# rockcarry/ffcnn

Measured on AMD Instinct MI355X. Metric: frames/sec yolo-fastest-1.1 @320x320 batch-64 per GPU (u8 BGR frames -> net_input's conversion in the first kernel -> full forward: conv stack + YOLO decode + NMS, boxes on rank 0), higher is better.
Workload: dtype f32

## Files before the change

ffcnn_amd/csrc/ffgpu_conv_kernels.inc:

```
#include "ffgpu_dw_stream.inc"
#include "ffgpu_pw_mfma.inc"
#include "ffgpu_pw_gemm32.inc"
#include "ffgpu_pw_bf16.inc"
#include "ffgpu_conv_igemm.inc"
#include "ffgpu_dwpw.inc"
#include "ffgpu_conv_dense.inc"
#include "ffgpu_irb.inc"
#include "ffgpu_irb_thin.inc"
#include "ffgpu_front.inc"
#include "ffgpu_irb_wave.inc"
#include "ffgpu_irb_wave2.inc"
#include "ffgpu_pw_x3.inc"
#include "ffgpu_pw_x3t.inc"
#include "ffgpu_conv_x3.inc"
#include "ffgpu_dw_lds.inc"
#include "ffgpu_dw_pair.inc"
#include "ffgpu_conv_thin.inc"

struct BareScratch {
    float *p = nullptr; size_t n = 0; int dev = -1;
    float *get(size_t need)
    {
        int d = 0;
        (void)hipGetDevice(&d);
// ... 1079 lines not shown
            const long tiles = (long)((d.OW + 4 * TWq - 1) / (4 * TWq)) * ((d.OH + TH - 1) / TH);
            const double cost = (double)tiles * (NSI * (c.KS1 * 128.0 + 500.0) + 4 * (220.0 + c.OT * 128.0)) * (1.0 + 12.0 / EW);
            if (cost < best) { best = cost; c.TWq = TWq; c.TH = TH; c.EW = EW; c.EH = EH; c.NSI = NSI; }
        }
    }
    if (best > 1e29) return false;
    const int ft = env_int("FFGPU_IRBW_TWQ", 0), fh = env_int("FFGPU_IRBW_TH", 0);
    if (ft > 0 && fh > 0 && ft * fh <= 16) {
        const int EW = S == 1 ? 4 * ft + 4 : 8 * ft + 4, EH = S * (fh - 1) + 3;
        if (EW * EH <= c.NSI * 64) { c.TWq = ft; c.TH = fh; c.EW = EW; c.EH = EH; }
    }
    const long ntiles = (long)d.N * ((d.OW + 4 * c.TWq - 1) / (4 * c.TWq)) * ((d.OH + c.TH - 1) / c.TH);
    const int regs = c.NSI * c.KS1 * 4 + c.OT * 16 + 2 * (c.KS1 + 4 * c.OT) + 76;
    c.big = regs > 124;
    if (env_int("FFGPU_IRBW_BIG", -1) >= 0) c.big = env_int("FFGPU_IRBW_BIG", -1) != 0;
    if (S == 2 && c.KS1 == 1 && env_int("FFGPU_IRBW_BIG_S2K1", -1) >= 0) c.big = env_int("FFGPU_IRBW_BIG_S2K1", -1) != 0;
    const bool conc = (d.flags & FFGPU_CONCURRENT) != 0;
    const int gmax = std::min(8, c.ngroups);
    int G = 1;
    for (int g = 1; g <= gmax; g++) {
        const size_t slot = (size_t)c.OT * 1024, ereg = (size_t)g * 16 * c.NSI * 64;
        if (g > 1 && ereg / slot < (size_t)(g + 1) / 2) continue;
        G = g;
        if (ntiles * g >= env_int("FFGPU_IRBW_GWAVES", conc ? 500 : 1200)) break;
    }
    if (!conc && G > 1 && G < gmax && c.ngroups % G != 0 && (c.ngroups + G) / (G + 1) <= (c.ngroups + G - 1) / G) G++;
    if (d.stride == 1 && c.ngroups == 9 && ntiles >= 400 && ntiles < 512 && gmax >= 4 && !conc && !env_int("FFGPU_IRBW_NOEXC", 0)) G = 4;
    if (ntiles >= 256 && ntiles < 1100 && env_int("FFGPU_IRBW_G_MID", 0) > 0) G = std::min(gmax, env_int("FFGPU_IRBW_G_MID", 0));
    const bool xl_ok = S == 1 && c.KS1 == 12 && c.OT == 3 && c.NSI == 2 && c.big && ((env_int("FFGPU_IRBW_X3", 30) >> 3) & 1) != 0;
    if (xl_ok && conc && ntiles < 256) G = std::min(gmax, env_int("FFGPU_IRBW_G_XL", 7));
    if (ntiles < 256 && env_int("FFGPU_IRBW_G_SMALL", 0) > 0) G = std::min(gmax, env_int("FFGPU_IRBW_G_SMALL", 0));
    const int fg = env_int("FFGPU_IRBW_G", 0);
    if (fg >= 1 && fg <= gmax) G = fg;
    c.G = G;
    c.NSO = 1;
    c.x3 = S == 1 && c.KS1 == 6 && c.OT == 2 && c.NSI == 2 && c.big && ((env_int("FFGPU_IRBW_X3", 30) >> 2) & 1) != 0;
    if (S == 2 && c.KS1 == 4 && c.OT == 2 && c.NSI == 4 && c.big && ((env_int("FFGPU_IRBW_X3", 30) >> 4) & 1) != 0) c.x3 = true;
    c.xl = xl_ok && G > 1;
    if (c.xl) c.x3 = true;
    if (G == 1 && S == 1 && c.OT == 1 && (c.KS1 == 2 || c.KS1 == 4) && env_int("FFGPU_IRBW_NSO", 2) == 2) {
        double best2 = 1e30; int tw2 = 0, th2 = 0;
        for (int TWq = 1; TWq <= 8; TWq++) {
            if (TWq > 1 && (TWq - 1) * 4 >= d.OW) break;
            for (int TH = 1; TWq * TH <= 32 && TH <= d.OH + 1; TH++) {
                if (TWq * TH <= 16 || TWq * ((TH + 1) / 2) > 16) continue;
                const int EW = 4 * TWq + 4, EH = TH + 2;
                if (EW * EH > 192) continue;
                const long tiles = (long)((d.OW + 4 * TWq - 1) / (4 * TWq)) * ((d.OH + TH - 1) / TH);
                const double cost = (double)tiles * (3 * (c.KS1 * 128.0 + 500.0) + 2 * 4 * (220.0 + 128.0)) * (1.0 + 12.0 / EW);
                if (cost < best2) { best2 = cost; tw2 = TWq; th2 = TH; }
            }
        }
        const int f2t = env_int("FFGPU_IRBW2_TWQ", 0), f2h = env_int("FFGPU_IRBW2_TH", 0);
        if (f2t > 0 && f2h > 0 && f2t * ((f2h + 1) / 2) <= 16 && (4 * f2t + 4) * (f2h + 2) <= 192) { tw2 = f2t; th2 = f2h; best2 = 0; }
        const long nt2 = tw2 ? (long)d.N * ((d.OW + 4 * tw2 - 1) / (4 * tw2)) * ((d.OH + th2 - 1) / th2) : 0;
        if (tw2 && best2 < 0.93 * best && nt2 >= env_int("FFGPU_IRBW2_MIN_TILES", 768)) {
            c.NSO = 2; c.TWq = tw2; c.TH = th2; c.EW = 4 * tw2 + 4; c.EH = th2 + 2; c.NSI = 3; c.big = true; c.WPB = 4; c.xl = false;
            c.x3 = irbw_x3_has(c.KS1) && ((env_int("FFGPU_IRBW_X3", 30) >> (c.KS1 == 2 ? 0 : 1)) & 1) != 0;
        }
    }
    {
        const size_t cs = ((size_t)c.ngroups * 224 + c.OT * 32) * sizeof(float), slice = (size_t)16 * c.NSI * 64 * sizeof(float);
        const int cap = c.big ? 12 : 16;
        const int w4 = std::min(cap, (int)(IRB_LDS_MAX / (cs + 4 * slice)) * 4), w8 = std::min(cap, (int)(IRB_LDS_MAX / (cs + 8 * slice)) * 8);
        c.WPB = G > 1 ? G : (w4 >= w8 ? 4 : 8);
        const int fw = env_int("FFGPU_IRBW_WPB", 0);
        if (G == 1 && fw >= 1 && fw <= 8) c.WPB = fw;
    }
    return true;
}

static int irbw_half(const IrbDesc &d, const IrbwCfg &c)
{
    const int r = d.ec & 15;
    const bool on = d.half ? d.half == 2 : env_int("FFGPU_IRBW_HALF", 1) != 0;
    return c.NSO == 1 && r >= 1 && r <= 8 && on ? 1 : 0;
}

static void irbw_layout(const IrbwCfg &c, int &o_w2, int &o_cs, int &cs_floats, int &total)
{
    o_w2 = c.x3 ? c.ngroups * irbw_x3_nm(c.KS1) * 256 : c.ngroups * c.KS1 * 64;
    o_cs = o_w2 + c.ngroups * 4 * c.OT * 64;
    cs_floats = c.ngroups * 16 * 14 + c.OT * 32;
    total = o_cs + cs_floats;
}

template <typename L>
static int irbw_traced(const IrbwP &p, long nblocks, hipStream_t s, L launch)
{
    {
        static unsigned long long *d_t = nullptr;
        if (!d_t && hipMalloc(&d_t, 4096 * 16 * sizeof(unsigned long long)) != hipSuccess) return -1;
        IrbwP q = p; q.dbg_t = d_t;
        (void)hipMemsetAsync(d_t, 0, 4096 * 16 * sizeof(unsigned long long), s);
        launch(q);
        (void)hipStreamSynchronize(s);
        const long nb = std::min(nblocks, 4096L);
        std::vector<unsigned long long> h((size_t)nb * 16);
        (void)hipMemcpy(h.data(), d_t, h.size() * sizeof(unsigned long long), hipMemcpyDeviceToHost);
        unsigned long long t0 = ~0ull, t1 = 0; double d[5] = { 0 }, ex[6] = { 0 }; double late = 0;
        for (long b = 0; b < nb; b++) { t0 = std::min(t0, h[b * 16]); t1 = std::max(t1, h[b * 16 + 5]); }
        for (long b = 0; b < nb; b++) {
            late = std::max(late, (double)(h[b * 16] - t0) * 0.01);
            d[0] += (double)(h[b * 16 + 1] - h[b * 16]) / nb * 0.01; d[1] += (double)(h[b * 16 + 2] - h[b * 16 + 1]) / nb * 0.01;
            d[2] += (double)(h[b * 16 + 3] - h[b * 16 + 2]) / nb * 0.01;
            const unsigned long long t4 = h[b * 16 + 4] ? h[b * 16 + 4] : h[b * 16 + 3];
            d[3] += (double)(t4 - h[b * 16 + 3]) / nb * 0.01; d[4] += (double)(h[b * 16 + 5] - t4) / nb * 0.01;
            for (int k = 0; k < 6; k++) ex[k] += (double)h[b * 16 + 8 + k] / nb * 0.01;
        }
        fprintf(stderr, "  trace irbw %dx%d %d->%d->%d: span %.2f us (first %ld blocks), last start +%.2f | issue loads %.2f barrier %.2f groups %.2f [expand mfma %.2f store %.2f dw0 %.2f prj0 %.2f dw1 %.2f prj1 %.2f] reduce %.2f rows %.2f (us, wave 0, mean per workgroup)\n",
                p.W, p.H, p.ic, p.ec, p.oc, (double)(t1 - t0) * 0.01, nb, late, d[0], d[1], d[2], ex[0], ex[1], ex[2], ex[3], ex[4], ex[5], d[3], d[4]);
        return 0;
    }
}

template <int KS1, int OT, int S, int NSI, bool BIG>
static int irbw_launch_t(const IrbwP &p, size_t lds, long nblocks, int threads, hipStream_t s)
{
    if (lds_allow((const void *)k_irbw<KS1, OT, S, NSI, BIG>, lds, "irbw")) return -1;
    if (env_int("FFGPU_IRB_TRACE", 0))
        return irbw_traced(p, nblocks, s, [&](const IrbwP &q) { hipLaunchKernelGGL((k_irbw<KS1, OT, S, NSI, BIG>), dim3((unsigned)nblocks), dim3(threads), lds, s, q); });
    hipLaunchKernelGGL((k_irbw<KS1, OT, S, NSI, BIG>), dim3((unsigned)nblocks), dim3(threads), lds, s, p);
    LAUNCH_OK("irbw");
    return 0;
}

static int launch_irbw(const IrbDesc &d, const IrbwCfg &c, hipStream_t s)
{
    auto slope = [](int act) { return act == 2 ? 0.1f : (act == 1 ? 0.f : 1.f); };
    IrbwP p;
    p.in = d.in; p.out = d.out; p.residual = d.residual; p.pk = d.pk;
    p.N = d.N; p.H = d.H; p.W = d.W; p.OH = d.OH; p.OW = d.OW; p.ic = d.ic; p.ec = d.ec; p.oc = d.oc;
    p.act1 = slope(d.act1); p.actd = slope(d.actd); p.act2 = slope(d.act2); p.res_act = slope(d.res_act);
    p.TWq = c.TWq; p.TH = c.TH; p.EW = c.EW; p.EH = c.EH;
    p.tiles_x = (d.OW + 4 * c.TWq - 1) / (4 * c.TWq); p.tiles_y = (d.OH + c.TH - 1) / c.TH;
    p.ntiles = (long)d.N * p.tiles_x * p.tiles_y;
    p.ngroups = c.ngroups; p.G = c.G; p.WPB = c.WPB;
    p.half_last = irbw_half(d, c);
    { const int x = env_int("FFGPU_IRBW_XCD", 3); p.xcd = c.G > 1 ? (x >> 1) & 1 : x & 1; }
    int total;
    irbw_layout(c, p.o_w2, p.o_cs, p.cs_floats, total);
    size_t region = (size_t)(c.G > 1 ? c.G : c.WPB) * 16 * c.NSI * 64;
    if (c.G > 1 && !env_int("FFGPU_IRBW_FOLD", 0)) {
        const size_t want = (size_t)c.G * c.OT * 1024;
        if (want > region && (p.cs_floats + want) * sizeof(float) <= 150 * 1024 && p.ntiles <= 512) region = want;
    }
    p.red_cap = (int)(region / ((size_t)c.OT * 1024));
    p.in_elems = (unsigned)((size_t)d.ic * d.N * d.H * d.W);
    p.vec = d.OW % 4 == 0 ? 4 : (d.OW % 2 == 0 ? 2 : 1);
    p.m_ew = (unsigned)(((1ULL << 32) + c.EW - 1) / c.EW);
    {
        auto magic = [](long dv) { return dv <= 1 ? 0u : (unsigned)(((1ULL << 32) + (unsigned long long)dv - 1) / (unsigned long long)dv); };
        if (p.ntiles * std::max(p.tiles_x, p.tiles_y) >= (1L << 32) || p.ntiles >= (1L << 31)) { ffgpu_set_error("irbw: too many tiles for 32-bit index arithmetic"); return -1; }
        p.m_tx = magic(p.tiles_x); p.m_ty = magic(p.tiles_y); p.m_twq = magic(p.TWq);
    }
    p.dbg_t = nullptr;
    const int waves = c.G > 1 ? c.G : c.WPB;
    p.xl_off = (int)((size_t)p.cs_floats + region);
    const size_t lds = ((size_t)p.cs_floats + region + (c.xl ? (size_t)c.NSI * 4 * 64 * IRBW_XL_DW : 0)) * sizeof(float);
    const long nblocks = c.G > 1 ? p.ntiles : (p.ntiles + c.WPB - 1) / c.WPB;
    if (env_int("FFGPU_VERBOSE_IRB", 0))
        fprintf(stderr, "irbw %dx%d %d->%d->%d s%d: tile %dx%d halo %dx%d (%d strips, %d out), %d groups, G %d, %ld tiles, %ld blocks x %d waves, lds %zu B%s\n",
                d.W, d.H, d.ic, d.ec, d.oc, d.stride, 4 * c.TWq, c.TH, c.EW, c.EH, c.NSI, c.NSO, c.ngroups, c.G, p.ntiles, nblocks, waves, lds, c.big ? ", 256 VGPR" : "");
    if (c.NSO == 2) {
        if (c.KS1 == 2 && c.x3)  { hipLaunchKernelGGL((k_irbw2<2, 3, true>), dim3((unsigned)nblocks), dim3(waves * 64), lds, s, p); LAUNCH_OK("irbw2"); return 0; }
        if (c.KS1 == 4 && c.x3)  { hipLaunchKernelGGL((k_irbw2<4, 3, true>), dim3((unsigned)nblocks), dim3(waves * 64), lds, s, p); LAUNCH_OK("irbw2"); return 0; }
        if (c.KS1 == 2) { hipLaunchKernelGGL((k_irbw2<2, 3, false>), dim3((unsigned)nblocks), dim3(waves * 64), lds, s, p); LAUNCH_OK("irbw2"); return 0; }
        if (c.KS1 == 4) { hipLaunchKernelGGL((k_irbw2<4, 3, false>), dim3((unsigned)nblocks), dim3(waves * 64), lds, s, p); LAUNCH_OK("irbw2"); return 0; }
    }
    if (c.xl && c.NSO == 1) {
        if (lds_allow((const void *)k_irbw<12, 3, 1, 2, true, true, true>, lds, "irbw")) return -1;
        if (env_int("FFGPU_IRB_TRACE", 0))
            return irbw_traced(p, nblocks, s, [&](const IrbwP &q) { hipLaunchKernelGGL((k_irbw<12, 3, 1, 2, true, true, true>), dim3((unsigned)nblocks), dim3(waves * 64), lds, s, q); });
        hipLaunchKernelGGL((k_irbw<12, 3, 1, 2, true, true, true>), dim3((unsigned)nblocks), dim3(waves * 64), lds, s, p);
        LAUNCH_OK("irbw");
        return 0;
    }
    if (c.x3 && c.NSO == 1 && c.KS1 == 4 && c.OT == 2 && d.stride == 2 && c.NSI == 4) {
        if (lds_allow((const void *)k_irbw<4, 2, 2, 4, true, true>, lds, "irbw")) return -1;
        if (env_int("FFGPU_IRB_TRACE", 0))
            return irbw_traced(p, nblocks, s, [&](const IrbwP &q) { hipLaunchKernelGGL((k_irbw<4, 2, 2, 4, true, true>), dim3((unsigned)nblocks), dim3(waves * 64), lds, s, q); });
        hipLaunchKernelGGL((k_irbw<4, 2, 2, 4, true, true>), dim3((unsigned)nblocks), dim3(waves * 64), lds, s, p);
        LAUNCH_OK("irbw");
        return 0;
    }
    if (c.x3 && c.NSO == 1 && c.KS1 == 6 && c.OT == 2 && d.stride == 1 && c.NSI == 2) {
        if (lds_allow((const void *)k_irbw<6, 2, 1, 2, true, true>, lds, "irbw")) return -1;
        if (env_int("FFGPU_IRB_TRACE", 0))
            return irbw_traced(p, nblocks, s, [&](const IrbwP &q) { hipLaunchKernelGGL((k_irbw<6, 2, 1, 2, true, true>), dim3((unsigned)nblocks), dim3(waves * 64), lds, s, q); });
        hipLaunchKernelGGL((k_irbw<6, 2, 1, 2, true, true>), dim3((unsigned)nblocks), dim3(waves * 64), lds, s, p);
        LAUNCH_OK("irbw");
        return 0;
    }
#define IRBW_CASE(ks1, ot, st, nsi) if (c.KS1 == ks1 && c.OT == ot && d.stride == st && c.NSI == nsi) \
        return c.big ? irbw_launch_t<ks1, ot, st, nsi, true>(p, lds, nblocks, waves * 64, s) : irbw_launch_t<ks1, ot, st, nsi, false>(p, lds, nblocks, waves * 64, s);
    IRBW_CASE(1, 1, 1, 2); IRBW_CASE(2, 1, 1, 2); IRBW_CASE(4, 1, 1, 2); IRBW_CASE(2, 2, 1, 2); IRBW_CASE(4, 2, 1, 2); IRBW_CASE(6, 2, 1, 2); IRBW_CASE(12, 3, 1, 2);
// ... 55 lines not shown
    LAUNCH_OK("front");
    return 0;
}

bool ffgpu_irb_supported(const IrbDesc &d)
{
    if (irb_thin_ok(d)) return true;
    { IrbwCfg c; if (irbw_pick(d, c)) return true; }
    if (d.stride != 1 && d.stride != 2) return false;
    if (d.oc > 48 || d.ic > 64 || d.ec < 1) return false;
    if (d.act1 == 3 || d.actd == 3 || d.act2 == 3 || d.res_act == 3) return false;
    if (((long)d.H * d.W) % 4 || ((long)d.OH * d.OW) % 4) return false;
    IrbP p;
    return irb_pick_tile(d, p);
}

static void irb_consts(const IrbDesc &d, int &k4, int &ECH, int &MT, int &OT, int &nchunks, int &CH)
{
    k4 = (d.ic + 3) & ~3; OT = (d.oc + 15) / 16;
    ECH = irb_ech(d); MT = ECH / 16;
    nchunks = (d.ec + ECH - 1) / ECH;
    CH = irb_chunk_floats(k4, ECH, OT);
}

size_t ffgpu_irb_pack_floats(const IrbDesc &d)
{
    if (irb_thin_ok(d)) return 64;
    { IrbwCfg c; if (irbw_pick(d, c)) { int a, b, cs, total; irbw_layout(c, a, b, cs, total); return (size_t)total; } }
    int k4, ECH, MT, OT, nchunks, CH;
    irb_consts(d, k4, ECH, MT, OT, nchunks, CH);
    return ((size_t)nchunks * CH + OT * 32 + 63) & ~(size_t)63;
}

void ffgpu_irb_plan(IrbDesc &d) { d.half = env_int("FFGPU_IRBW_HALF", 1) != 0 ? 2 : 1; }

int ffgpu_irb_pack(const IrbDesc &d, float *pk, hipStream_t s)
{
    if (irb_thin_ok(d)) return 0;
    { IrbwCfg c;
      if (irbw_pick(d, c)) {
          int a, b, cs, total; irbw_layout(c, a, b, cs, total);
          IrbwPackP q; q.w1 = d.w1; q.wd = d.wd; q.w2 = d.w2; q.pk = pk; q.ic = d.ic; q.ec = d.ec; q.oc = d.oc;
          q.k4 = (d.ic + 3) & ~3; q.OT = c.OT; q.ngroups = c.ngroups; q.x3 = c.x3 ? 1 : 0; q.half = irbw_half(d, c);
          hipLaunchKernelGGL(k_irbw_pack, dim3((total + 255) / 256), dim3(256), 0, s, q);
          LAUNCH_OK("irbw_pack");
          return 0;
      } }
    IrbPackP q;
    q.w1 = d.w1; q.wd = d.wd; q.w2 = d.w2; q.pk = pk;
    q.ic = d.ic; q.ec = d.ec; q.oc = d.oc;
    irb_consts(d, q.k4, q.ECH, q.MT, q.OT, q.nchunks, q.CH);
    const int total = q.nchunks * q.CH + q.OT * 32;
    hipLaunchKernelGGL(k_irb_pack, dim3((total + 255) / 256), dim3(256), 0, s, q);
    LAUNCH_OK("irb_pack");
    return 0;
}

template <int MT, int OT, int S, int SPW, int NW>
static int irb_launch_t(const IrbP &p, size_t lds, long nblocks, hipStream_t s)
{
    if (lds_allow((const void *)k_irb<MT, OT, SPW, S, NW>, lds, "irb")) return -1;
    if (env_int("FFGPU_IRB_TRACE", 0)) {
        static unsigned long long *d_t = nullptr;
        if (!d_t && hipMalloc(&d_t, 4096 * 16 * sizeof(unsigned long long)) != hipSuccess) return -1;
        IrbP q = p; q.dbg_t = d_t;
        (void)hipMemsetAsync(d_t, 0, 4096 * 16 * sizeof(unsigned long long), s);
        hipLaunchKernelGGL((k_irb<MT, OT, SPW, S, NW>), dim3((unsigned)nblocks), dim3(NW * 64), lds, s, q);
        (void)hipStreamSynchronize(s);
        std::vector<unsigned long long> h((size_t)nblocks * 16);
        (void)hipMemcpy(h.data(), d_t, h.size() * sizeof(unsigned long long), hipMemcpyDeviceToHost);
        unsigned long long t0 = ~0ull, t1 = 0; double d[7] = { 0 }, ph[4] = { 0 };
        for (long b = 0; b < nblocks; b++) {
            t0 = std::min(t0, h[b * 16]); t1 = std::max(t1, h[b * 16 + 7]);
            for (int k = 0; k < 7; k++) d[k] += (double)(h[b * 16 + k + 1] - h[b * 16 + k]) / nblocks * 0.01;
            for (int k = 0; k < 4; k++) ph[k] += (double)h[b * 16 + 8 + k] / nblocks * 0.01;
        }
// ... 61 lines not shown
```

ffcnn_amd/csrc/ffgpu_dev.hpp:

```cpp
#pragma once
#include <hip/hip_runtime.h>
#include <stddef.h>
#include <stdint.h>
#include <vector>
#include "ffgpu_internal.h"

#define FFGPU_CHECK(expr)                                                                   \
    do {                                                                                    \
        hipError_t e_ = (expr);                                                             \
        if (e_ != hipSuccess) {                                                             \
            ffgpu_set_error("%s failed: %s (%s:%d)", #expr, hipGetErrorString(e_), __FILE__, __LINE__); \
            return -1;                                                                      \
        }                                                                                   \
    } while (0)

struct ConvDesc {
    const float *in;
    const float *const *in_ind;
    const float *filt;
    float       *out;
    const float *residual;
    const float *wpack;
    int   N;
    int   iw, ih, ic;
    int   ow, oh, oc;
    int   fs, stride, pad, groups;
    int   act;
    int   res_act;
    int   flags;
    long  in_cs, in_ns, out_cs, out_ns, res_cs, res_ns;
    int   nsplit;
    int   kernel;
    int   x3_mt;
};
#define FFGPU_F_BATCH_INPUT (1 << 30)

static inline int conv_k4(const ConvDesc &d) { return (d.fs * d.fs * (d.ic / d.groups) + 3) & ~3; }

struct IrbDesc {
    const float *in; float *out; const float *residual;
    const float *w1, *wd, *w2;
    int N, H, W, OH, OW, ic, ec, oc, stride;
    int act1, actd, act2, res_act;
    const float *pk;
    int flags;
    int half;
};
bool   ffgpu_irb_supported(const IrbDesc &d);
bool   ffgpu_irb_is_thin(const IrbDesc &d);
size_t ffgpu_irb_pack_floats(const IrbDesc &d);
void   ffgpu_irb_plan(IrbDesc &d);
int    ffgpu_irb_pack(const IrbDesc &d, float *pk, hipStream_t s);
int    ffgpu_launch_irb(const IrbDesc &d, hipStream_t s);
bool   ffgpu_front_ok(const ConvDesc &c, const IrbDesc &d);
enum InputForm { IN_F32, IN_U8, IN_BGR_FRAMES, IN_NV12_FRAMES, IN_FORMS };
int    ffgpu_launch_front(const ConvDesc &c, const IrbDesc &d, InputForm form, hipStream_t s);
bool   ffgpu_front_nv12_fused();
int    ffgpu_front_nc(const IrbDesc &d);

bool   ffgpu_dwpw_ok(const ConvDesc &dw, const ConvDesc &pw);
size_t ffgpu_dwpw_pack_floats(const ConvDesc &dw, const ConvDesc &pw);
int    ffgpu_dwpw_pack(const ConvDesc &dw, const ConvDesc &pw, float *pk, hipStream_t s);
int    ffgpu_launch_dwpw(const ConvDesc &dw, const ConvDesc &pw, const float *wpack, hipStream_t s);

size_t ffgpu_pw_pack_floats(const ConvDesc &d);
void   ffgpu_conv_plan(ConvDesc &d);
int    ffgpu_pw_pack(const ConvDesc &d, float *pk, hipStream_t s);

struct FrameDesc {
    const unsigned char *bgr;
    int w, h, pitch;
    int sw, sh, s1, s2;
    int fmt;
    const unsigned char *uv;
    int pitch_uv;
    int pad_;
};
static_assert(sizeof(FrameDesc) == 56, "FrameDesc: 64 of them travel by value as k_set_frames' argument");
#define FFGPU_YUV_MATRICES { { 16, 298, 409, 100, 208, 516 }, { 0, 256, 359, 88, 183, 454 }, { 16, 298, 459, 55, 136, 541 }, { 0, 256, 403, 48, 120, 475 } }
// ... 50 lines not shown
```

ffcnn_amd/csrc/ffgpu_irb_wave.inc:

```
typedef float v4f_w __attribute__((ext_vector_type(4)));
typedef float v2f_w __attribute__((ext_vector_type(2)));

struct IrbwP {
    const float *in; float *out; const float *residual;
    const float *pk;
    int N, H, W, OH, OW, ic, ec, oc;
    float act1, actd, act2, res_act;
    int TWq, TH, EW, EH;
    int tiles_x, tiles_y;
    long ntiles;
    int ngroups, G, WPB;
    int o_w2, o_cs;
    int cs_floats;
    int xl_off;
    int red_cap;
    unsigned in_elems;
    int vec;
    int half_last;
    unsigned m_ew;
    unsigned m_tx, m_ty, m_twq;
    int xcd;
    unsigned long long *dbg_t;
};

__device__ __forceinline__ int irbw_xcd_block(int b, int nb) { const int q = nb >> 3, r = nb & 7, x = b & 7; return x * q + min(x, r) + (b >> 3); }
__device__ __forceinline__ int irbw_div(int i, unsigned m) { return m ? (int)__umulhi((unsigned)i, m) : i; }

struct IrbwPackP {
    const float *w1, *wd, *w2; float *pk;
    int ic, ec, oc, k4, OT, ngroups;
    int x3;
    int half;
};
__host__ __device__ __forceinline__ int irbw_chan(int pos, int ngroups, int half)
{
    const int g = pos >> 4, rho = pos & 15;
    return (half && g == ngroups - 1) ? 16 * g + (rho >> 2) + 4 * (rho & 3) : pos;
}

#include "ffgpu_x3_terms.h"
static bool irbw_x3_has(int ks1) { return ks1 == 2 || ks1 == 4 || ks1 == 6 || ks1 == 12; }
#ifndef X3_INF_EXACT
#define X3_INF_EXACT 1
#endif
#ifndef X3_INF_W
#define X3_INF_W X3_INF_EXACT
#endif
#ifndef X3_INF_X
#define X3_INF_X X3_INF_EXACT
#endif
#ifndef X3_INF_X_FUSED
#define X3_INF_X_FUSED X3_INF_X
#endif
#ifndef X3_INF_X_CONV
#define X3_INF_X_CONV X3_INF_X
#endif
__device__ __forceinline__ float x3_resid(float x)
{
#if X3_WHATIF_NOSPLIT
    return 0.f;
#endif
    const float r = x - __uint_as_float(__float_as_uint(x) & 0xffff0000u);
#if X3_INF_X
    return __builtin_amdgcn_classf(x, 0x204) ? 0.f : r;
#else
// ... 37 lines not shown
    const unsigned u1 = __float_as_uint(r) & 0xffff0000u;
    unsigned v = (part == 1 ? u1 : __float_as_uint(r - __uint_as_float(u1))) >> 16;
#if X3_INF_W
    const unsigned ex = (uw >> 23) & 0xffu;
    if ((v & 0x7fffu) == 0 && ex >= 41u && ex != 255u) v = ((uw >> 16) & 0x8000u) | ((ex - 40u) << 7);
#endif
    return v;
}

__global__ void k_irbw_pack(IrbwPackP p)
{
    const int ks1 = p.k4 >> 2, ecp = p.ngroups * 16, nm = irbw_x3_nm(ks1);
    const int n1 = p.x3 ? p.ngroups * nm * 256 : p.ngroups * ks1 * 64, n2 = p.ngroups * 4 * p.OT * 64, n3 = ecp * 12, n4 = ecp * 2, n5 = p.OT * 32;
    const int rl1 = p.k4 + 4, rl2 = ((p.ec + 3) & ~3) + 4;
    for (int i = blockIdx.x * blockDim.x + threadIdx.x; i < n1 + n2 + n3 + n4 + n5; i += gridDim.x * blockDim.x) {
        float v = 0.f;
        int j = i;
        if (j < n1 && p.x3) {
            const int d = j & 3, l = (j >> 2) & 63, m = (j >> 8) % nm, g = (j >> 8) / nm;
            const int e = irbw_chan(16 * g + (l & 15), p.ngroups, p.half), kq = l >> 4;
            const IrbwX3Term t = irbw_x3_term(ks1, m, d);
            unsigned bits = 0;
            if (t.wp >= 0 && e < p.ec) {
                const float wa = p.w1[(long)e * rl1 + 4 * (2 * t.pair) + kq], wb = p.w1[(long)e * rl1 + 4 * (2 * t.pair + 1) + kq];
                bits = irbw_x3_part(wa, t.wp) | (irbw_x3_part(wb, t.wp) << 16);
            }
            v = __uint_as_float(bits);
        } else if (j < n1) {
            const int l = j & 63, ks = (j >> 6) % ks1, g = (j >> 6) / ks1;
            const int e = irbw_chan(16 * g + (l & 15), p.ngroups, p.half), ci = 4 * ks + (l >> 4);
            if (e < p.ec) v = p.w1[(long)e * rl1 + ci];
        } else if ((j -= n1) < n2) {
            const int l = j & 63, t = (j >> 6) % p.OT, ks = ((j >> 6) / p.OT) & 3, g = (j >> 6) / (p.OT * 4);
            const int o = 16 * t + (l & 15), e = irbw_chan(16 * g + 4 * (l >> 4) + ks, p.ngroups, p.half);
            if (o < p.oc && e < p.ec) v = p.w2[(long)o * rl2 + e];
        } else if ((j -= n2) < n3) {
            const int pr = j / 24, k = (j % 24) >> 1, e = irbw_chan(2 * pr + (j & 1), p.ngroups, p.half);
            if (e < p.ec && k < 11) v = k < 9 ? p.wd[(long)e * 16 + k] : p.wd[(long)e * 16 + 12 + (k - 9)];
        } else if ((j -= n3) < n4) {
            const int e = irbw_chan(4 * (j >> 3) + (j & 3), p.ngroups, p.half);
            if (e < p.ec) v = p.w1[(long)e * rl1 + p.k4 + ((j >> 2) & 1)];
        } else {
            j -= n4;
            const int o = j >> 1;
            if (o < p.oc) v = p.w2[(long)o * rl2 + (rl2 - 4) + (j & 1)];
        }
        p.pk[i] = v;
    }
}

typedef unsigned u4_w2 __attribute__((ext_vector_type(4)));
typedef __bf16 v8bf_w2 __attribute__((ext_vector_type(8)));
template <class T> __device__ __forceinline__ T irbw_ld(const void *base, unsigned byte_off)
{ return *reinterpret_cast<const T *>(reinterpret_cast<const char *>(base) + byte_off); }
template <class T> __device__ __forceinline__ void irbw_st(void *base, unsigned byte_off, T v)
{ *reinterpret_cast<T *>(reinterpret_cast<char *>(base) + byte_off) = v; }
__device__ __forceinline__ float irbw_act(float x, float slope) { return fmaxf(x, slope * x); }

template <int KS1, int OT, int S, int NSI, bool BIG, bool X3 = false, bool XL = false>
#ifndef IRBW_MID_WAVES
#define IRBW_MID_WAVES 3
#endif
__global__ void __launch_bounds__(512, BIG ? 2 : (KS1 == 1 && OT == 1 && S == 2 && NSI == 3 ? IRBW_MID_WAVES : 4)) k_irbw(IrbwP p)
{
    static_assert(!XL || (X3 && KS1 == 12), "XL: the LDS-resident split tile exists for 48 input channels");
    constexpr int NM = X3 ? irbw_x3_nm(KS1) : 1;
    struct W1T { float f[X3 ? 1 : KS1]; u4_w2 x[X3 ? NM : 1]; };
#if IRB_TRACE
#define IRBW_T(k) do { if (p.dbg_t && threadIdx.x == 0 && blockIdx.x < 4096) p.dbg_t[blockIdx.x * 16 + (k)] = __builtin_amdgcn_s_memrealtime(); } while (0)
#else
#define IRBW_T(k) do { } while (0)
#endif
    IRBW_T(0);
    extern __shared__ __attribute__((aligned(16))) float smem[];
    const int tid = threadIdx.x, lane = tid & 63, wid = __builtin_amdgcn_readfirstlane(tid >> 6);
    const int kq = lane >> 4, jq = lane & 15;
    constexpr int NPw = NSI * 64, NQ = NSI * 16;
    constexpr bool PIPE = !X3 && BIG && NSI * 16 + NSI * KS1 * 4 + OT * 16 + 2 * (KS1 + 4 * OT) <= 140;
    const int ecp = p.ngroups * 16;
    const float *Wd = smem, *Sb1 = smem + ecp * 12, *Sb2 = Sb1 + ecp * 2;
    float *Ew = smem + p.cs_floats + wid * (16 * NPw);
    const v4f_w z = { 0.f, 0.f, 0.f, 0.f };

    const int cs4 = p.cs_floats >> 2, nthr = (int)blockDim.x;
    v4f_w cst[3];
#pragma unroll
    for (int u = 0; u < 3; u++) cst[u] = irbw_ld<v4f_w>(p.pk, (unsigned)(p.o_cs + 4 * min(tid + u * nthr, cs4 - 1)) * 4u);

    const int bid = p.xcd ? irbw_xcd_block((int)blockIdx.x, (int)gridDim.x) : (int)blockIdx.x;
    const int tile = p.G > 1 ? bid : bid * p.WPB + wid;
    const bool active = tile < (int)p.ntiles;
    const int tt = active ? tile : 0;
    const int trow = irbw_div(tt, p.m_tx), tx_i = tt - trow * p.tiles_x;
    const int n = irbw_div(trow, p.m_ty), ty_i = trow - n * p.tiles_y;
    const int oy0 = ty_i * p.TH, ox0 = tx_i * p.TWq * 4;
    const int gy0 = oy0 * S - 1, gx0 = ox0 * S - 1;
    const bool interior = gy0 >= 0 && gx0 >= 0 && gy0 + p.EH <= p.H && gx0 + p.EW <= p.W;

    v4f_w xin[XL ? 1 : NSI][KS1];
    unsigned mbits = 0;
    const int plane = p.H * p.W;
    auto load_strip = [&](int si, v4f_w (&x)[KS1]) {
        const int e = si * 64 + 4 * jq;
        const int iy = (int)__umulhi((unsigned)e, p.m_ew), ix = e - iy * p.EW;
        const int rowidx = (n * p.H + min(max(gy0 + iy, 0), p.H - 1)) * p.W + gx0 + ix;
        bool anyfix = false;
#pragma unroll
        for (int ks = 0; ks < KS1; ks++) {
            const int idx = min(4 * ks + kq, p.ic - 1) * (p.N * plane) + rowidx;
// ... 71 lines not shown
    }
    unsigned xp[X3 && !XL ? NSI : 1][4][3][X3 && !XL ? KS1 / 2 : 1];
    if (X3 && !XL) {
        float amax = 0.f;
#pragma unroll
        for (int si = 0; si < NSI; si++)
#pragma unroll
            for (int ks = 0; ks < KS1; ks++) amax = x3_amax3(x3_amax3(amax, xin[si][ks][0], xin[si][ks][1]), xin[si][ks][2], xin[si][ks][3]);
        auto split_tile = [&](auto INF) {
#pragma unroll
            for (int si = 0; si < NSI; si++)
#pragma unroll
                for (int q = 0; q < 4; q++) {
                    unsigned b[3][KS1];
#pragma unroll
                    for (int ks = 0; ks < KS1; ks++) split3(INF, xin[si][ks][q], b[0][ks], b[1][ks], b[2][ks]);
#pragma unroll
                    for (int pt = 0; pt < 3; pt++)
#pragma unroll
                        for (int pr = 0; pr < KS1 / 2; pr++) xp[si][q][pt][pr] = __builtin_amdgcn_perm(b[pt][2 * pr + 1], b[pt][2 * pr], 0x07060302u);
                }
        };
        if (X3_INF_X_FUSED && x3_wave_has_inf(amax)) split_tile(std::true_type{}); else split_tile(std::false_type{});
    }
    auto bop = [&](int si, int q, int m) -> v8bf_w2 {
        u4_w2 u;
#pragma unroll
        for (int d = 0; d < 4; d++) {
            const IrbwX3Term t = irbw_x3_term(KS1, m, d);
            u[d] = t.wp < 0 ? 0u : xp[X3 && !XL ? si : 0][q][t.xp][X3 && !XL ? t.pair : 0];
        }
        return __builtin_bit_cast(v8bf_w2, u);
    };
    const int ty = irbw_div(jq, p.m_twq), tq = jq - ty * p.TWq;
    const bool qvalid = ty < p.TH;
    const int ebase = qvalid ? ty * S * p.EW + tq * 4 * S : 0;

    const int oy = oy0 + ty, ox = ox0 + tq * 4;
    const bool valid = active && qvalid && oy < p.OH && ox < p.OW;
    const int nvalid = valid ? min(4, p.OW - ox) : 0;
    const unsigned pbase = valid ? (unsigned)((n * p.OH + oy) * p.OW + ox) : 0u;
    const unsigned ocs = (unsigned)(p.N * p.OH * p.OW);
    auto res_issue = [&](int t, int r) -> v4f_w {
        const unsigned off = ((unsigned)min(16 * t + 4 * kq + r, p.oc - 1) * ocs + pbase) * 4u;
        v4f_w v;
        if (p.vec == 4) v = irbw_ld<v4f_w>(p.residual, nvalid == 4 ? off : 0u);
        else if (p.vec == 2) {
            const v2f_w a = irbw_ld<v2f_w>(p.residual, nvalid >= 2 ? off : 0u), b = irbw_ld<v2f_w>(p.residual, nvalid == 4 ? off + 8u : 0u);
            v = (v4f_w){ a.x, a.y, b.x, b.y };
        } else {
#pragma unroll
            for (int q = 0; q < 4; q++) v[q] = irbw_ld<float>(p.residual, q < nvalid ? off + 4u * q : 0u);
        }
        return v;
    };
    constexpr bool RPRE = OT == 1 && KS1 <= 2;
    v4f_w rpre[4];
    if (RPRE && p.G == 1 && p.residual) {
#pragma unroll
        for (int r = 0; r < 4; r++) rpre[r] = res_issue(0, r);
    }
    auto loadw1 = [&](int g, W1T &w1) {
        if (X3) {
#pragma unroll
            for (int m = 0; m < NM; m++) w1.x[m] = irbw_ld<u4_w2>(p.pk, (unsigned)((g * NM + m) * 64 + lane) * 16u);
        } else {
#pragma unroll
            for (int ks = 0; ks < KS1; ks++) w1.f[ks] = irbw_ld<float>(p.pk, (unsigned)((g * KS1 + ks) * 64 + lane) * 4u);
        }
    };
    auto loadw = [&](int g, W1T &w1, float (&w2)[4 * OT]) {
        loadw1(g, w1);
// ... 104 lines not shown
            const float *row = ep + r * p.EW;
            constexpr int NX = S == 1 ? 6 : 9;
            v2f_w x[NX + 1];
#pragma unroll
            for (int i = 0; i < NX / 2; i++) {
                const v4f_w u = *reinterpret_cast<const v4f_w *>(row + ((i & 1) * NQ + (i >> 1)) * 4);
                x[2 * i] = (v2f_w){ u.x, u.y }; x[2 * i + 1] = (v2f_w){ u.z, u.w };
            }
            if (NX & 1) x[NX - 1] = *reinterpret_cast<const v2f_w *>(row + ((NX - 1) >> 2) * 4);
#pragma unroll
            for (int q = 0; q < 4; q++)
#pragma unroll
                for (int kx = 0; kx < 3; kx++) dv[q] += tap[r * 3 + kx] * x[S * q + kx];
        }
#pragma unroll
        for (int q = 0; q < 4; q++) {
            const v2f_w t = dv[q] * sd + bd;
            const v2f_w u = t * p.actd;
            bq[q] = (v2f_w){ fmaxf(t.x, u.x), fmaxf(t.y, u.y) };
        }
    };
    auto project = [&](const float (&w2)[4 * OT], int m, const v2f_w (&bq)[4]) {
#pragma unroll
        for (int j = 0; j < 2; j++)
#pragma unroll
            for (int t = 0; t < OT; t++) {
                const float a = w2[(2 * m + j) * OT + t];
                acc[t][0] = __builtin_amdgcn_mfma_f32_16x16x4f32(a, j ? bq[0].y : bq[0].x, acc[t][0], 0, 0, 0);
                acc[t][1] = __builtin_amdgcn_mfma_f32_16x16x4f32(a, j ? bq[1].y : bq[1].x, acc[t][1], 0, 0, 0);
                acc[t][2] = __builtin_amdgcn_mfma_f32_16x16x4f32(a, j ? bq[2].y : bq[2].x, acc[t][2], 0, 0, 0);
                acc[t][3] = __builtin_amdgcn_mfma_f32_16x16x4f32(a, j ? bq[3].y : bq[3].x, acc[t][3], 0, 0, 0);
            }
    };
    auto loadw2 = [&](int g, float (&w2)[4 * OT]) {
#pragma unroll
        for (int i = 0; i < 4 * OT; i++) w2[i] = irbw_ld<float>(p.pk, (unsigned)(p.o_w2 + (g * 4 * OT + i) * 64 + lane) * 4u);
    };
    const int ngw = gfirst < p.ngroups ? (p.ngroups - gfirst + gstep - 1) / gstep : 0;
    auto gi = [&](int i) { return min(gfirst + i * gstep, p.ngroups - 1); };

    if (active && ngw > 0) {
        if (PIPE) {
            v4f_w a4[NSI][4];
            v2f_w bq0[4], bq1[4];
            loadw1(gi(1), w1b);
            expand_mfma(w1a, a4);
            expand_store(gi(0), a4);
            auto body = [&](int i, W1T &w1cur, float (&w2cur)[4 * OT], W1T &w1nxt, float (&w2nxt)[4 * OT]) {
                loadw2(gi(i + 1), w2nxt);
                __builtin_amdgcn_sched_barrier(0);
                expand_mfma(w1nxt, a4);
                dw_stage(gi(i), 0, bq0);
                if (!halfg(gi(i))) dw_stage(gi(i), 1, bq1);
                __builtin_amdgcn_sched_barrier(0);
                loadw1(gi(i + 2), w1cur);
                project(w2cur, 0, bq0);
                if (!halfg(gi(i))) project(w2cur, 1, bq1);
                expand_store(gi(i + 1), a4);
                __builtin_amdgcn_sched_barrier(0);
            };
            auto tail = [&](int i, float (&w2cur)[4 * OT]) {
                dw_stage(gi(i), 0, bq0);
                project(w2cur, 0, bq0);
                if (halfg(gi(i))) return;
                dw_stage(gi(i), 1, bq1);
                project(w2cur, 1, bq1);
            };
            int i = 0;
            for (; i + 2 < ngw; i += 2) { body(i, w1a, w2a, w1b, w2b); body(i + 1, w1b, w2b, w1a, w2a); }
            if (i + 1 < ngw) { body(i, w1a, w2a, w1b, w2b); tail(i + 1, w2b); } else tail(i, w2a);
        } else {
            v4f_w a4[NSI][4];
            v2f_w bq[4];
#if IRB_TRACE
            unsigned long long tph[6] = { 0, 0, 0, 0, 0, 0 };
#define IRBW_TP(k) do { __builtin_amdgcn_sched_barrier(0); const unsigned long long tn_ = __builtin_amdgcn_s_memrealtime(); tph[k] += tn_ - tq0; tq0 = tn_; __builtin_amdgcn_sched_barrier(0); } while (0)
#else
#define IRBW_TP(k) do { } while (0)
#endif
            auto group = [&](int g, const W1T &w1, const float (&w2)[4 * OT]) {
#if IRB_TRACE
                unsigned long long tq0 = __builtin_amdgcn_s_memrealtime();
#endif
                expand_mfma(w1, a4);
                IRBW_TP(0);
                expand_store(g, a4);
                IRBW_TP(1);
                dw_stage(g, 0, bq);
                IRBW_TP(2);
                project(w2, 0, bq);
                IRBW_TP(3);
                if (halfg(g)) return;
                dw_stage(g, 1, bq);
                IRBW_TP(4);
                project(w2, 1, bq);
                IRBW_TP(5);
            };
            if (X3) {
                auto group_x3 = [&](int g, int gnext, const float (&w2)[4 * OT]) {
                    if (NSI > 2) {
#pragma unroll
                        for (int si = 0; si < NSI; si++) { expand_strip(si, w1a, a4[0]); store_strip(g, si, a4[0]); }
                        __builtin_amdgcn_sched_barrier(0);
                        loadw1(gnext, w1a);
                    } else {
                        expand_mfma(w1a, a4);
                        __builtin_amdgcn_sched_barrier(0);
                        loadw1(gnext, w1a);
                        expand_store(g, a4);
                    }
                    dw_stage(g, 0, bq);
                    project(w2, 0, bq);
                    if (halfg(g)) return;
                    dw_stage(g, 1, bq);
                    project(w2, 1, bq);
                };
                for (int i = 0; i < ngw; i += 2) {
                    loadw2(gi(i + 1), w2b);
                    __builtin_amdgcn_sched_barrier(0);
                    group_x3(gi(i), gi(i + 1), w2a);
                    if (i + 1 < ngw) {
                        loadw2(gi(i + 2), w2a);
                        __builtin_amdgcn_sched_barrier(0);
                        group_x3(gi(i + 1), gi(i + 2), w2b);
                    }
                }
            } else
            for (int i = 0; i < ngw; i += 2) {
                loadw1(gi(i + 1), w1b); loadw2(gi(i + 1), w2b);
                __builtin_amdgcn_sched_barrier(0);
                group(gi(i), w1a, w2a);
                if (i + 1 < ngw) {
                    loadw1(gi(i + 2), w1a); loadw2(gi(i + 2), w2a);
                    __builtin_amdgcn_sched_barrier(0);
                    group(gi(i + 1), w1b, w2b);
                }
            }
#if IRB_TRACE
            if (p.dbg_t && threadIdx.x == 0 && blockIdx.x < 4096) for (int k = 0; k < 6; k++) p.dbg_t[blockIdx.x * 16 + 8 + k] = tph[k];
#endif
#undef IRBW_TP
        }
    }

    IRBW_T(3);
    const bool lin_out = p.act2 == 1.f && p.res_act == 1.f;
    auto row_out = [&](int t, int r, v4f_w v, v4f_w res) {
        const int o = 16 * t + 4 * kq + r, oo = min(o, p.oc - 1);
        const float sc = Sb2[2 * oo], bi = Sb2[2 * oo + 1];
        if (lin_out) {
#pragma unroll
            for (int q = 0; q < 4; q++) { v[q] = fmaf(v[q], sc, bi); if (p.residual) v[q] += res[q]; }
        } else {
#pragma unroll
            for (int q = 0; q < 4; q++) {
                v[q] = irbw_act(fmaf(v[q], sc, bi), p.act2);
                if (p.residual) v[q] = irbw_act(v[q] + res[q], p.res_act);
            }
        }
        const unsigned off = ((unsigned)oo * ocs + pbase) * 4u;
        if (o < p.oc) {
            if (p.vec == 4) { if (nvalid == 4) irbw_st<v4f_w>(p.out, off, v); }
            else if (p.vec == 2) {
                if (nvalid >= 2) irbw_st<v2f_w>(p.out, off, (v2f_w){ v.x, v.y });
                if (nvalid == 4) irbw_st<v2f_w>(p.out, off + 8u, (v2f_w){ v.z, v.w });
            } else {
#pragma unroll
                for (int q = 0; q < 4; q++) if (q < nvalid) irbw_st<float>(p.out, off + 4u * q, v[q]);
            }
        }
    };

    if (p.G == 1) {
        if (RPRE) {
#pragma unroll
            for (int r = 0; r < 4; r++)
                row_out(0, r, (v4f_w){ acc[0][0][r], acc[0][1][r], acc[0][2][r], acc[0][3][r] }, rpre[r]);
// ... 88 lines not shown
```

Baseline: 197,900.

## Pair depthwise strips into one MFMA projection for small-output stride-2 IRB

For stride-2 inverted-residual blocks with at most 8 output channels and small tiles, the two halves of each group's depthwise output are processed by separate half-waves. Each half-wave computes one strip, and a single merged projection MFMA pass consumes both. A cross-lane bpermute then sums the partial accumulators. The packed projection weights are re-laid out so output rows 8-15 hold the second strip's weights. The goal is to halve the depthwise and projection instruction count on MFMA lanes that were wasted on padded output channels, at the cost of an extra reduction shuffle and a forced G=1.

```diff
diff --git a/ffcnn_amd/csrc/ffgpu_conv_kernels.inc b/ffcnn_amd/csrc/ffgpu_conv_kernels.inc
--- a/ffcnn_amd/csrc/ffgpu_conv_kernels.inc
+++ b/ffcnn_amd/csrc/ffgpu_conv_kernels.inc
@@ -1135,6 +1135,7 @@
     if (ntiles < 256 && env_int("FFGPU_IRBW_G_SMALL", 0) > 0) G = std::min(gmax, env_int("FFGPU_IRBW_G_SMALL", 0));
     const int fg = env_int("FFGPU_IRBW_G", 0);
     if (fg >= 1 && fg <= gmax) G = fg;
+    if (d.pair == 2) G = 1;
     c.G = G;
     c.NSO = 1;
     c.x3 = S == 1 && c.KS1 == 6 && c.OT == 2 && c.NSI == 2 && c.big && ((env_int("FFGPU_IRBW_X3", 30) >> 2) & 1) != 0;
@@ -1178,6 +1179,13 @@
     const int r = d.ec & 15;
     const bool on = d.half ? d.half == 2 : env_int("FFGPU_IRBW_HALF", 1) != 0;
     return c.NSO == 1 && r >= 1 && r <= 8 && on ? 1 : 0;
+}
+
+static int irbw_pair(const IrbDesc &d, const IrbwCfg &c)
+{
+    if (d.pair) return d.pair == 2;
+    return d.stride == 2 && c.OT == 1 && d.oc <= 8 && c.NSI == 3 && c.NSO == 1 && c.G == 1 && !c.x3 && c.TWq * c.TH <= 8 &&
+           env_int("FFGPU_IRBW_S2PAIR", 1) != 0;
 }
 
 static void irbw_layout(const IrbwCfg &c, int &o_w2, int &o_cs, int &cs_floats, int &total)
@@ -1240,6 +1248,8 @@
     p.ntiles = (long)d.N * p.tiles_x * p.tiles_y;
     p.ngroups = c.ngroups; p.G = c.G; p.WPB = c.WPB;
     p.half_last = irbw_half(d, c);
+    p.pair = irbw_pair(d, c);
+    if (p.pair && (d.stride != 2 || c.OT != 1 || c.NSI != 3 || c.G != 1 || c.x3 || c.TWq * c.TH > 8)) { ffgpu_set_error("irbw: the planned paired-column form does not fit this launch"); return -1; }
     { const int x = env_int("FFGPU_IRBW_XCD", 3); p.xcd = c.G > 1 ? (x >> 1) & 1 : x & 1; }
     int total;
     irbw_layout(c, p.o_w2, p.o_cs, p.cs_floats, total);
@@ -1263,8 +1273,9 @@
     const size_t lds = ((size_t)p.cs_floats + region + (c.xl ? (size_t)c.NSI * 4 * 64 * IRBW_XL_DW : 0)) * sizeof(float);
     const long nblocks = c.G > 1 ? p.ntiles : (p.ntiles + c.WPB - 1) / c.WPB;
     if (env_int("FFGPU_VERBOSE_IRB", 0))
-        fprintf(stderr, "irbw %dx%d %d->%d->%d s%d: tile %dx%d halo %dx%d (%d strips, %d out), %d groups, G %d, %ld tiles, %ld blocks x %d waves, lds %zu B%s\n",
-                d.W, d.H, d.ic, d.ec, d.oc, d.stride, 4 * c.TWq, c.TH, c.EW, c.EH, c.NSI, c.NSO, c.ngroups, c.G, p.ntiles, nblocks, waves, lds, c.big ? ", 256 VGPR" : "");
+        fprintf(stderr, "irbw %dx%d %d->%d->%d s%d: tile %dx%d halo %dx%d (%d strips, %d out), %d groups, G %d, %ld tiles, %ld blocks x %d waves, lds %zu B%s%s\n",
+                d.W, d.H, d.ic, d.ec, d.oc, d.stride, 4 * c.TWq, c.TH, c.EW, c.EH, c.NSI, c.NSO, c.ngroups, c.G, p.ntiles, nblocks, waves, lds, c.big ? ", 256 VGPR" : "",
+                p.pair ? ", paired columns" : "");
     if (c.NSO == 2) {
         if (c.KS1 == 2 && c.x3)  { hipLaunchKernelGGL((k_irbw2<2, 3, true>), dim3((unsigned)nblocks), dim3(waves * 64), lds, s, p); LAUNCH_OK("irbw2"); return 0; }
         if (c.KS1 == 4 && c.x3)  { hipLaunchKernelGGL((k_irbw2<4, 3, true>), dim3((unsigned)nblocks), dim3(waves * 64), lds, s, p); LAUNCH_OK("irbw2"); return 0; }
@@ -1386,7 +1397,13 @@
     return ((size_t)nchunks * CH + OT * 32 + 63) & ~(size_t)63;
 }
 
-void ffgpu_irb_plan(IrbDesc &d) { d.half = env_int("FFGPU_IRBW_HALF", 1) != 0 ? 2 : 1; }
+void ffgpu_irb_plan(IrbDesc &d)
+{
+    d.half = env_int("FFGPU_IRBW_HALF", 1) != 0 ? 2 : 1;
+    d.pair = 0;
+    IrbwCfg c;
+    d.pair = !irb_thin_ok(d) && irbw_pick(d, c) && irbw_pair(d, c) ? 2 : 1;
+}
 
 int ffgpu_irb_pack(const IrbDesc &d, float *pk, hipStream_t s)
 {
@@ -1395,7 +1412,7 @@
       if (irbw_pick(d, c)) {
           int a, b, cs, total; irbw_layout(c, a, b, cs, total);
           IrbwPackP q; q.w1 = d.w1; q.wd = d.wd; q.w2 = d.w2; q.pk = pk; q.ic = d.ic; q.ec = d.ec; q.oc = d.oc;
-          q.k4 = (d.ic + 3) & ~3; q.OT = c.OT; q.ngroups = c.ngroups; q.x3 = c.x3 ? 1 : 0; q.half = irbw_half(d, c);
+          q.k4 = (d.ic + 3) & ~3; q.OT = c.OT; q.ngroups = c.ngroups; q.x3 = c.x3 ? 1 : 0; q.half = irbw_half(d, c); q.pair = irbw_pair(d, c);
           hipLaunchKernelGGL(k_irbw_pack, dim3((total + 255) / 256), dim3(256), 0, s, q);
           LAUNCH_OK("irbw_pack");
           return 0;
diff --git a/ffcnn_amd/csrc/ffgpu_dev.hpp b/ffcnn_amd/csrc/ffgpu_dev.hpp
--- a/ffcnn_amd/csrc/ffgpu_dev.hpp
+++ b/ffcnn_amd/csrc/ffgpu_dev.hpp
@@ -45,6 +45,7 @@
     const float *pk;
     int flags;
     int half;
+    int pair;
 };
 bool   ffgpu_irb_supported(const IrbDesc &d);
 bool   ffgpu_irb_is_thin(const IrbDesc &d);
diff --git a/ffcnn_amd/csrc/ffgpu_irb_wave.inc b/ffcnn_amd/csrc/ffgpu_irb_wave.inc
--- a/ffcnn_amd/csrc/ffgpu_irb_wave.inc
+++ b/ffcnn_amd/csrc/ffgpu_irb_wave.inc
@@ -17,6 +17,7 @@
     unsigned in_elems;
     int vec;
     int half_last;
+    int pair;
     unsigned m_ew;
     unsigned m_tx, m_ty, m_twq;
     int xcd;
@@ -31,6 +32,7 @@
     int ic, ec, oc, k4, OT, ngroups;
     int x3;
     int half;
+    int pair;
 };
 __host__ __device__ __forceinline__ int irbw_chan(int pos, int ngroups, int half)
 {
@@ -134,7 +136,14 @@
             if (e < p.ec) v = p.w1[(long)e * rl1 + ci];
         } else if ((j -= n1) < n2) {
             const int l = j & 63, t = (j >> 6) % p.OT, ks = ((j >> 6) / p.OT) & 3, g = (j >> 6) / (p.OT * 4);
-            const int o = 16 * t + (l & 15), e = irbw_chan(16 * g + 4 * (l >> 4) + ks, p.ngroups, p.half);
+            int o = 16 * t + (l & 15), pos = 16 * g + 4 * (l >> 4) + ks;
+            if (p.pair) {
+                const int i = l & 15, up = i >> 3, hg = p.half && g == p.ngroups - 1;
+                o = i & 7;
+                pos = 16 * g + 4 * (l >> 4) + (hg ? up : 2 * up + ks);
+                if (ks >= (hg ? 1 : 2)) o = p.oc;
+            }
+            const int e = irbw_chan(pos, p.ngroups, p.half);
             if (o < p.oc && e < p.ec) v = p.w2[(long)o * rl2 + e];
         } else if ((j -= n2) < n3) {
             const int pr = j / 24, k = (j % 24) >> 1, e = irbw_chan(2 * pr + (j & 1), p.ngroups, p.half);
@@ -177,6 +186,8 @@
     extern __shared__ __attribute__((aligned(16))) float smem[];
     const int tid = threadIdx.x, lane = tid & 63, wid = __builtin_amdgcn_readfirstlane(tid >> 6);
     const int kq = lane >> 4, jq = lane & 15;
+    constexpr bool PAIRC = S == 2 && OT == 1 && NSI == 3 && !X3;
+    const bool pairf = PAIRC && p.pair != 0;
     constexpr int NPw = NSI * 64, NQ = NSI * 16;
     constexpr bool PIPE = !X3 && BIG && NSI * 16 + NSI * KS1 * 4 + OT * 16 + 2 * (KS1 + 4 * OT) <= 140;
     const int ecp = p.ngroups * 16;
@@ -314,12 +325,13 @@
         }
         return __builtin_bit_cast(v8bf_w2, u);
     };
-    const int ty = irbw_div(jq, p.m_twq), tq = jq - ty * p.TWq;
+    const int jo = pairf ? jq & 7 : jq;
+    const int ty = irbw_div(jo, p.m_twq), tq = jo - ty * p.TWq;
     const bool qvalid = ty < p.TH;
     const int ebase = qvalid ? ty * S * p.EW + tq * 4 * S : 0;
 
     const int oy = oy0 + ty, ox = ox0 + tq * 4;
-    const bool valid = active && qvalid && oy < p.OH && ox < p.OW;
+    const bool valid = active && qvalid && oy < p.OH && ox < p.OW && !(pairf && jq >= 8);
     const int nvalid = valid ? min(4, p.OW - ox) : 0;
     const unsigned pbase = valid ? (unsigned)((n * p.OH + oy) * p.OW + ox) : 0u;
     const unsigned ocs = (unsigned)(p.N * p.OH * p.OW);
@@ -490,6 +502,18 @@
                 acc[t][3] = __builtin_amdgcn_mfma_f32_16x16x4f32(a, j ? bq[3].y : bq[3].x, acc[t][3], 0, 0, 0);
             }
     };
+    auto project_pair = [&](const float (&w2)[4 * OT], bool hg, const v2f_w (&bq)[4]) {
+        if (hg) {
+            const bool up = jq >= 8;
+#pragma unroll
+            for (int q = 0; q < 4; q++) acc[0][q] = __builtin_amdgcn_mfma_f32_16x16x4f32(w2[0], up ? bq[q].y : bq[q].x, acc[0][q], 0, 0, 0);
+            return;
+        }
+#pragma unroll
+        for (int j = 0; j < 2; j++)
+#pragma unroll
+            for (int q = 0; q < 4; q++) acc[0][q] = __builtin_amdgcn_mfma_f32_16x16x4f32(w2[j * OT], j ? bq[q].y : bq[q].x, acc[0][q], 0, 0, 0);
+    };
     auto loadw2 = [&](int g, float (&w2)[4 * OT]) {
 #pragma unroll
         for (int i = 0; i < 4 * OT; i++) w2[i] = irbw_ld<float>(p.pk, (unsigned)(p.o_w2 + (g * 4 * OT + i) * 64 + lane) * 4u);
@@ -508,6 +532,16 @@
                 loadw2(gi(i + 1), w2nxt);
                 __builtin_amdgcn_sched_barrier(0);
                 expand_mfma(w1nxt, a4);
+                if (PAIRC && pairf) {
+                    const bool hg = halfg(gi(i));
+                    dw_stage(gi(i), hg ? 0 : jq >> 3, bq0);
+                    __builtin_amdgcn_sched_barrier(0);
+                    loadw1(gi(i + 2), w1cur);
+                    project_pair(w2cur, hg, bq0);
+                    expand_store(gi(i + 1), a4);
+                    __builtin_amdgcn_sched_barrier(0);
+                    return;
+                }
                 dw_stage(gi(i), 0, bq0);
                 if (!halfg(gi(i))) dw_stage(gi(i), 1, bq1);
                 __builtin_amdgcn_sched_barrier(0);
@@ -518,6 +552,12 @@
                 __builtin_amdgcn_sched_barrier(0);
             };
             auto tail = [&](int i, float (&w2cur)[4 * OT]) {
+                if (PAIRC && pairf) {
+                    const bool hg = halfg(gi(i));
+                    dw_stage(gi(i), hg ? 0 : jq >> 3, bq0);
+                    project_pair(w2cur, hg, bq0);
+                    return;
+                }
                 dw_stage(gi(i), 0, bq0);
                 project(w2cur, 0, bq0);
                 if (halfg(gi(i))) return;
@@ -544,6 +584,14 @@
                 IRBW_TP(0);
                 expand_store(g, a4);
                 IRBW_TP(1);
+                if (PAIRC && pairf) {
+                    const bool hg = halfg(g);
+                    dw_stage(g, hg ? 0 : jq >> 3, bq);
+                    IRBW_TP(2);
+                    project_pair(w2, hg, bq);
+                    IRBW_TP(3);
+                    return;
+                }
                 dw_stage(g, 0, bq);
                 IRBW_TP(2);
                 project(w2, 0, bq);
@@ -601,6 +649,13 @@
         }
     }
 
+    if (PAIRC && pairf) {
+        const int src = ((lane + 40) & 63) * 4;
+#pragma unroll
+        for (int q = 0; q < 4; q++)
+#pragma unroll
+            for (int r = 0; r < 4; r++) acc[0][q][r] += __int_as_float(__builtin_amdgcn_ds_bpermute(src, __float_as_int(acc[0][q][r])));
+    }
     IRBW_T(3);
     const bool lin_out = p.act2 == 1.f && p.res_act == 1.f;
     auto row_out = [&](int t, int r, v4f_w v, v4f_w res) {
```

Result: no change. 199,300, median of 6 (+0.7%).
